# lightonai/next-plaid

Measured on AMD Instinct MI355X. Metric: queries/sec + p50 latency, k=10, 10M-doc x 300-tok x d128 PLAID index, 1/2/4/8 GPU, higher is better.
Workload: dtype f32 (split-bf16 hi/lo MFMA on the residual term of MaxSim, f32-class accuracy)

## Files before the change

### next-plaid_amd/csrc/np_kernels.h

```cpp
#pragma once
#include <hip/hip_runtime.h>
#include <stdint.h>

namespace np {

typedef float f32x16 __attribute__((ext_vector_type(16)));
typedef __bf16 bf16x8 __attribute__((ext_vector_type(8)));

#define NP_NEG_INF (-__builtin_huge_valf())
#define NP_MAX_QT 8

__device__ __forceinline__ uint32_t okey(float x) {
  uint32_t b = __float_as_uint(x);
  uint32_t k = (b & 0x80000000u) ? ~b : (b | 0x80000000u);
  return ((b & 0x7F800000u) == 0x7F800000u) ? 0u : k;
}
__device__ __forceinline__ float unkey(uint32_t k) {
  uint32_t b = (k & 0x80000000u) ? (k ^ 0x80000000u) : ~k;
  return __uint_as_float(b);
}
__device__ __forceinline__ bool finitef(float x) { return (__float_as_uint(x) & 0x7F800000u) != 0x7F800000u; }
__device__ __forceinline__ float readlane_f(float v, int lane) {
  return __int_as_float(__builtin_amdgcn_readlane(__float_as_int(v), lane));
}
// ... 2011 lines not shown
    const uint4* metab = cand_meta + pbase;
    for (int64_t tile0 = 0; tile0 < n; tile0 += NG * NP_S4S_MAXD) {
      const int d = (int)min((int64_t)NP_S4S_MAXD, (n - tile0 + NG - 1) / NG);
      __syncthreads();
      for (int k = 0; k < d; ++k) {
        const int64_t i = tile0 + (int64_t)k * NG + gid;
        s_state[k][tid] = make_float4(NP_NEG_INF, NP_NEG_INF, NP_NEG_INF, NP_NEG_INF);
        if (jq == 0) {
          int64_t off = 0;
          uint4 sg = make_uint4(0, 0, 0, 0);
          if (i < n) {
            const uint4 m = metab[i];
            off = (int64_t)m.z | ((int64_t)(m.w & 0xFF) << 32);
            sg = useg[m.x];
            toks += (unsigned long long)(m.w >> 8);
            ucnt += (unsigned long long)m.y;
          }
          s_off[k][g] = off;
          *reinterpret_cast<uint4*>(&s_end[k][g][0]) = sg;
        }
      }
      __syncthreads();
      for (int p = 0; p < P; ++p) {
        int len = 0;
        int64_t abs0 = 0;
        if (jq < d) {
          const int e = (int)s_end[jq][g][((p + 1) << pshift) - 1];
          const int s = p ? (int)s_end[jq][g][(p << pshift) - 1] : 0;
          len = e - s;
          abs0 = s_off[jq][g] + s;
        }
        const int pad = (len + 3) & ~3;
        int incl = pad;
#pragma unroll
        for (int o = 1; o < LPR; o <<= 1) {
          const int v = __shfl_up(incl, o, LPR);
          if (jq >= o) incl += v;
        }
        if (jq < NP_S4S_MAXD) {
          s_pfx[g][jq] = incl - pad;
          s_abs[g][jq] = abs0;
          s_len[g][jq] = len;
        }
        const int Lg = __shfl(incl, lbase + LPR - 1);
        int maxL = Lg;
#pragma unroll
        for (int o = LPR; o < 64; o <<= 1) maxL = max(maxL, __shfl_xor(maxL, o));
        maxL = __builtin_amdgcn_readfirstlane(maxL);
        __builtin_amdgcn_fence(__ATOMIC_RELEASE, "wavefront");
        __builtin_amdgcn_wave_barrier();
        const int p1 = s_pfx[g][1], p2 = s_pfx[g][2], p3 = s_pfx[g][3], p4 = s_pfx[g][4];
        const uint32_t slice_lo = (uint32_t)(p << pshift) * slice_w;
        const char* Tp = Tb + (size_t)slice_lo * row_bytes;
        for (int base = 0; base < maxL; base += NP_S4S_CAP) {
#pragma unroll
          for (int h = 0; h < 2; ++h) {
            uint32_t cv[NST / 2];
#pragma unroll
            for (int i = 0; i < NST / 2; ++i) {
              const int pos = base + jq + LPR * (h * (NST / 2) + i);
              const int slot = (pos >= p1) + (pos >= p2) + (pos >= p3) + (pos >= p4);
              const int idx = min(pos - s_pfx[g][slot], max(s_len[g][slot] - 1, 0));
              int64_t a = s_abs[g][slot] + (int64_t)max(idx, 0);
              a = (pos < Lg) ? min(a, T - 1) : 0;
              cv[i] = codes[a];
            }
#pragma unroll
            for (int i = 0; i < NST / 2; ++i) {
              const int w = jq + LPR * (h * (NST / 2) + i);
              const int pos = base + w;
              const bool valid = pos < Lg;
              const int slot = (pos >= p1) + (pos >= p2) + (pos >= p3) + (pos >= p4);
              s_codes[g][w] = valid ? (uint16_t)(cv[i] - slice_lo) : (uint16_t)0;
              if ((pos & 3) == 0) s_slot[g][w >> 2] = valid ? (uint8_t)slot : (uint8_t)NP_S4S_MAXD;
            }
          }
          __builtin_amdgcn_fence(__ATOMIC_RELEASE, "wavefront");
          __builtin_amdgcn_wave_barrier();
          const int nwin = min(NP_S4S_CAP, maxL - base);
          for (int t0 = 0; t0 < nwin; t0 += 8) {
            const bool two = t0 + 4 < nwin;
            const uint2 ca = *reinterpret_cast<const uint2*>(&s_codes[g][t0]);
            const int sa = (int)s_slot[g][t0 >> 2];
            float4 v[8];
            v[0] = *reinterpret_cast<const float4*>(Tp + ((ca.x & 0xFFFFu) * row_bytes + col_bytes));
            v[1] = *reinterpret_cast<const float4*>(Tp + ((ca.x >> 16) * row_bytes + col_bytes));
            v[2] = *reinterpret_cast<const float4*>(Tp + ((ca.y & 0xFFFFu) * row_bytes + col_bytes));
            v[3] = *reinterpret_cast<const float4*>(Tp + ((ca.y >> 16) * row_bytes + col_bytes));
            int sb = NP_S4S_MAXD;
            if (two) {
              const uint2 cb = *reinterpret_cast<const uint2*>(&s_codes[g][t0 + 4]);
              sb = (int)s_slot[g][(t0 + 4) >> 2];
              v[4] = *reinterpret_cast<const float4*>(Tp + ((cb.x & 0xFFFFu) * row_bytes + col_bytes));
              v[5] = *reinterpret_cast<const float4*>(Tp + ((cb.x >> 16) * row_bytes + col_bytes));
              v[6] = *reinterpret_cast<const float4*>(Tp + ((cb.y & 0xFFFFu) * row_bytes + col_bytes));
              v[7] = *reinterpret_cast<const float4*>(Tp + ((cb.y >> 16) * row_bytes + col_bytes));
            } else {
#pragma unroll
              for (int u = 4; u < 8; ++u) v[u] = make_float4(NP_NEG_INF, NP_NEG_INF, NP_NEG_INF, NP_NEG_INF);
            }
            s4_fence<8>(v);
            float4 ma = s_state[sa][tid];
#pragma unroll
            for (int u = 0; u < 4; ++u) {
              ma.x = fmaxf(ma.x, v[u].x);
              ma.y = fmaxf(ma.y, v[u].y);
              ma.z = fmaxf(ma.z, v[u].z);
              ma.w = fmaxf(ma.w, v[u].w);
            }
            s_state[sa][tid] = ma;
            float4 mb = s_state[sb][tid];
#pragma unroll
            for (int u = 4; u < 8; ++u) {
              mb.x = fmaxf(mb.x, v[u].x);
              mb.y = fmaxf(mb.y, v[u].y);
              mb.z = fmaxf(mb.z, v[u].z);
              mb.w = fmaxf(mb.w, v[u].w);
            }
            s_state[sb][tid] = mb;
          }
          __builtin_amdgcn_fence(__ATOMIC_RELEASE, "wavefront");
          __builtin_amdgcn_wave_barrier();
        }
      }
      for (int k = 0; k < d; ++k) {
        const int64_t i = tile0 + (int64_t)k * NG + gid;
        const float4 m = s_state[k][tid];
        float score = 0.f;
        for (int jj = 0; 4 * jj < lq; ++jj) {
          const float a0 = __shfl(m.x, lbase + jj), a1 = __shfl(m.y, lbase + jj);
          const float a2 = __shfl(m.z, lbase + jj), a3 = __shfl(m.w, lbase + jj);
          if (a0 > NP_NEG_INF) score += a0;
          if (4 * jj + 1 < lq && a1 > NP_NEG_INF) score += a1;
          if (4 * jj + 2 < lq && a2 > NP_NEG_INF) score += a2;
          if (4 * jj + 3 < lq && a3 > NP_NEG_INF) score += a3;
        }
        if (jq == 0 && i < n) approx[pbase + i] = s_end[k][g][7] ? score : 0.f;
      }
    }
  }
#pragma unroll
  for (int o = 32; o > 0; o >>= 1) {
    toks += __shfl_xor(toks, o);
    ucnt += __shfl_xor(ucnt, o);
  }
  if (lane == 0 && toks && ctr) {
    atomicAdd(&ctr->n_cand_tokens, toks);
    atomicAdd(&ctr->n_cand_codes, ucnt);
  }
}

#define NP_UB_NBX 96

template <int ROWB, typename CT, int MODE, int FLOOR = 0>
__global__ void __launch_bounds__(256) approx_ub_kernel(const uint8_t* __restrict__ QCU, int64_t KP,
                                                        const uint4* __restrict__ cand_meta ,
                                                        const int32_t* __restrict__ n_begin ,
                                                        const int32_t* __restrict__ n_count ,
                                                        const int32_t* __restrict__ n_cand ,
                                                        RoundPlan rp, int round,
                                                        int max_rounds, const CT* __restrict__ codes ,
                                                        const uint32_t* __restrict__ qflag, int n_sel,
                                                        uint16_t* __restrict__ U ,
                                                        uint32_t* __restrict__ hist , int hshift,
                                                        uint32_t* __restrict__ cursor ,
                                                        int32_t* __restrict__ slots ,
                                                        int32_t* __restrict__ ticket , int B,
                                                        int steal_min ,
                                                        Counters* ctr, int count_tokens ,
                                                        int direct_wpq ,
                                                        int static_claims ,
                                                        const uint32_t* __restrict__ warmbits = nullptr ,
                                                        const uint32_t* __restrict__ lam2_b = nullptr ,
                                                        const int32_t* __restrict__ qoff = nullptr ) {
  static_assert(FLOOR == 0 || (MODE == 2 && ROWB <= 64), "the floored level: bounds-checked loads");
  constexpr bool WLDS = FLOOR && sizeof(CT) == 2;
  constexpr int LPD = ROWB / 16;
  constexpr int DPW = 64 / LPD;
  constexpr int CAP = sizeof(CT) == 2 ? 128 : 64;
  constexpr int CPS = CAP / 32;
  constexpr bool NT = MODE == 1, OOB = MODE == 2;
  static_assert(ROWB == 32 || ROWB == 64 || ROWB == 128 || ROWB == 256, "row = power-of-two bytes >= LQP");
  __shared__ uint32_t s_hist[NP_UB_BINS];
  __shared__ CT s_codes[4][DPW][CAP];
  __shared__ uint32_t s_warm[WLDS ? 2048 : 4];
  __shared__ int s_ndk[4][FLOOR ? DPW : 1];
  __shared__ int64_t s_cl[4][DPW];
  __shared__ int s_nd[4][DPW];
  const int tid = threadIdx.x, lane = tid & 63, wave = tid >> 6;
  const int jl = lane & (LPD - 1), grp = lane / LPD;
  const int x = blockIdx.x & 7;
  if (round >= rp.round_tab[2 * max_rounds]) return;
  const int rb = rp.round_tab[2 * round], re = rp.round_tab[2 * round + 1];
  unsigned long long toks = 0, ucnt = 0, ndoc = 0;
  const int half = lane >> 5, hl = lane & 31;
  __shared__ int s_q;
  for (int step = 0;; ++step) {
    __syncthreads();
    if (direct_wpq > 0) {
      if (step > 0) break;
      const int j = rb + (int)blockIdx.x / direct_wpq;
      if (j >= re) break;
      if (tid == 0) s_q = rp.order[j];
    } else if (tid == 0)
      s_q = xcd_next_query(slots, ticket, x, step, B, rp.order, rb, re, [&]() {
        int best = -3;
        if (static_claims) return best;
        int64_t most = steal_min;
        for (int j = rb; j < re; ++j) {
          const int b2 = rp.order[j];
          if (qflag[b2] || n_cand[b2] <= n_sel) continue;
          const int64_t n2 = n_count[b2];
          const int64_t left = n2 - (int64_t)__hip_atomic_load(&cursor[b2], __ATOMIC_RELAXED, __HIP_MEMORY_SCOPE_AGENT);
          if (left >= most) {
            most = left;
            best = b2;
          }
        }
        return best;
      });
    __syncthreads();
    const int b = __builtin_amdgcn_readfirstlane(s_q);
    if (b < 0) break;
    if (qflag[b] || n_cand[b] <= n_sel) continue;
    const int64_t first = n_begin ? n_begin[b] : 0;
    const int64_t n = n_count[b];
    if (n <= 0) continue;
    const int64_t pbase = rp.cand_base[b] + first;
    const uint4* metab = cand_meta + pbase;
    const char* Tb = reinterpret_cast<const char*>(QCU + (int64_t)b * KP * ROWB) + jl * 16;
    const uint64_t tb64 = reinterpret_cast<uint64_t>(QCU + (int64_t)b * KP * ROWB);
    const uint32_t tlo = (uint32_t)__builtin_amdgcn_readfirstlane((int)(uint32_t)tb64);
    const uint32_t thi = (uint32_t)__builtin_amdgcn_readfirstlane((int)(uint32_t)(tb64 >> 32));
    const __amdgpu_buffer_rsrc_t trs = __builtin_amdgcn_make_buffer_rsrc(
        reinterpret_cast<void*>(((uint64_t)thi << 32) | tlo), 0, (int)(KP * ROWB), 0x00020000);
    uint32_t* hb = hist ? hist + (int64_t)b * NP_UB_BINS : nullptr;
    __syncthreads();
    if (hb)
      for (int i = tid; i < NP_UB_BINS; i += 256) s_hist[i] = 0;
    uint32_t lam2 = 0;
    int Lq = 0;
    const uint32_t* wb = nullptr;
    if constexpr (FLOOR) {
      wb = warmbits + (int64_t)b * (KP >> 5);
      if constexpr (WLDS)
        for (int i = tid; i < 2048; i += 256) s_warm[i] = i < (int)(KP >> 5) ? wb[i] : 0u;
      lam2 = lam2_b[b];
      Lq = qoff[b + 1] - qoff[b];
    }
    __syncthreads();
    const int64_t NWS = direct_wpq > 0 ? (int64_t)direct_wpq * 4 : (int64_t)(gridDim.x >> 3) * 4;
    const int64_t gw = direct_wpq > 0 ? (int64_t)((int)blockIdx.x % direct_wpq) * 4 + wave : (int64_t)(blockIdx.x >> 3) * 4 + wave;
    int64_t istat = gw * DPW;
    uint32_t inext = 0;
    if (!static_claims && lane == 0) inext = atomicAdd(&cursor[b], (uint32_t)DPW);
    for (;;) {
      const int64_t i0 = static_claims ? istat : (int64_t)(uint32_t)__builtin_amdgcn_readfirstlane((int)inext);
      if (i0 >= n) break;
      istat += NWS * DPW;
      if (!static_claims && lane == 0) inext = atomicAdd(&cursor[b], (uint32_t)DPW);
      const int64_t i = i0 + grp;
      const bool valid = i < n;
      uint4 m;
      if constexpr (NT) {
        const uint32_t* mp = reinterpret_cast<const uint32_t*>(metab + (valid ? i : n - 1));
        m = make_uint4(__builtin_nontemporal_load(mp), __builtin_nontemporal_load(mp + 1), __builtin_nontemporal_load(mp + 2),
                       __builtin_nontemporal_load(mp + 3));
      } else {
        m = metab[valid ? i : n - 1];
      }
      const int nd = valid ? (int)m.y : 0;
      const int64_t cl = (int64_t)m.z | ((int64_t)(m.w & 0xFF) << 32);
      if (jl == 0) {
        s_cl[wave][grp] = cl;
        s_nd[wave][grp] = nd;
        if (valid) {
          toks += (unsigned long long)(m.w >> 8);
          if constexpr (!FLOOR) ucnt += (unsigned long long)nd;
          ++ndoc;
        }
      }
      int nmax = nd;
#pragma unroll
      for (int o = LPD; o < 64; o <<= 1) nmax = max(nmax, __shfl_xor(nmax, o));
      nmax = __builtin_amdgcn_readfirstlane(nmax);
      uint32_t st[16];
#pragma unroll
      for (int k = 0; k < 16; ++k) st[k] = 0;
      for (int p0 = 0; p0 < nmax; p0 += CAP) {
        __builtin_amdgcn_fence(__ATOMIC_RELEASE, "wavefront");
        __builtin_amdgcn_wave_barrier();
        constexpr int SB = DPW / 2 < 8 ? DPW / 2 : 8;
#pragma unroll 1
        for (int sb = 0; sb < DPW / 2; sb += SB) {
          uint32_t cv[SB][4], c0[SB], wvg[(FLOOR && !WLDS) ? SB : 1][CPS];
          int nds[SB];
#pragma unroll
          for (int j = 0; j < SB; ++j) {
            const int sl = 2 * (sb + j) + half;
            nds[j] = s_nd[wave][sl];
            const CT* cp = codes + s_cl[wave][sl];
            const int pos = min(p0 + CPS * hl, max(nds[j] - 1, 0) & ~(CPS - 1));
            if constexpr (NT) {
              c0[j] = (uint32_t)__builtin_nontemporal_load(cp);
#pragma unroll
              for (int k = 0; k < CPS; ++k) cv[j][k] = (uint32_t)__builtin_nontemporal_load(cp + pos + k);
            } else {
              c0[j] = (uint32_t)cp[0];
              const uint2 raw = *reinterpret_cast<const uint2*>(cp + pos);
              if constexpr (sizeof(CT) == 2) {
                cv[j][0] = raw.x & 0xFFFFu; cv[j][1] = raw.x >> 16; cv[j][2] = raw.y & 0xFFFFu; cv[j][3] = raw.y >> 16;
              } else {
                cv[j][0] = raw.x; cv[j][1] = raw.y;
              }
            }
          }
          if constexpr (FLOOR && !WLDS) {
            const uint32_t wlast = (uint32_t)(KP >> 5) - 1u;
#pragma unroll
            for (int j = 0; j < SB; ++j)
#pragma unroll
              for (int k = 0; k < CPS; ++k)
                wvg[j][k] = (p0 + CPS * hl + k < nds[j]) ? wb[min(cv[j][k] >> 5, wlast)] : 0u;
          }
#pragma unroll
          for (int j = 0; j < SB; ++j) {
            const int sl = 2 * (sb + j) + half;
            const int pos = p0 + CPS * hl;
            if constexpr (FLOOR) {
              uint32_t wv[CPS];
#pragma unroll
              for (int k = 0; k < CPS; ++k) {
                if constexpr (WLDS) wv[k] = s_warm[(cv[j][k] >> 5) & 0x7FFu];
                else wv[k] = wvg[j][k];
              }
              int base = 0;
              CT* dstc = &s_codes[wave][sl][0];
#pragma unroll
              for (int k = 0; k < CPS; ++k) {
                const bool kp = pos + k < nds[j] && ((wv[k] >> (cv[j][k] & 31u)) & 1u) != 0u;
                const unsigned long long bal = __ballot(kp);
                const uint32_t hm = half ? (uint32_t)(bal >> 32) : (uint32_t)bal;
                if (kp) dstc[base + (int)__popc(hm & ((1u << hl) - 1u))] = (CT)cv[j][k];
                base += (int)__popc(hm);
              }
              if (hl == 0) s_ndk[wave][sl] = base;
              __builtin_amdgcn_sched_barrier(0);
              continue;
            }
#pragma unroll
            for (int k = 0; k < CPS; ++k)
              if (pos + k >= nds[j]) cv[j][k] = c0[j];
            CT* dst = &s_codes[wave][sl][CPS * hl];
            if constexpr (sizeof(CT) == 2) {
              *reinterpret_cast<uint2*>(dst) = make_uint2(cv[j][0] | (cv[j][1] << 16), cv[j][2] | (cv[j][3] << 16));
            } else {
              *reinterpret_cast<uint2*>(dst) = make_uint2(cv[j][0], cv[j][1]);
            }
          }
        }
        __builtin_amdgcn_fence(__ATOMIC_RELEASE, "wavefront");
        __builtin_amdgcn_wave_barrier();
        int np = (min(CAP, nmax - p0) + 7) & ~7;
        int ndk = 0;
        if constexpr (FLOOR) {
          ndk = s_ndk[wave][grp];
          if (jl == 0 && valid) ucnt += (unsigned long long)ndk;
          int km = ndk;
#pragma unroll
          for (int o = LPD; o < 64; o <<= 1) km = max(km, __shfl_xor(km, o));
          np = (__builtin_amdgcn_readfirstlane(km) + 7) & ~7;
        }
        const CT* mine = &s_codes[wave][grp][0];
        auto issue = [&](int t, uint4 (&v)[8]) {
          uint32_t c[8];
          if constexpr (sizeof(CT) == 2) {
            const uint4 cw = *reinterpret_cast<const uint4*>(mine + t);
            c[0] = cw.x & 0xFFFFu; c[1] = cw.x >> 16; c[2] = cw.y & 0xFFFFu; c[3] = cw.y >> 16;
            c[4] = cw.z & 0xFFFFu; c[5] = cw.z >> 16; c[6] = cw.w & 0xFFFFu; c[7] = cw.w >> 16;
          } else {
            const uint4 ca = *reinterpret_cast<const uint4*>(mine + t), cb = *reinterpret_cast<const uint4*>(mine + t + 4);
            c[0] = ca.x; c[1] = ca.y; c[2] = ca.z; c[3] = ca.w;
            c[4] = cb.x; c[5] = cb.y; c[6] = cb.z; c[7] = cb.w;
          }
          if constexpr (OOB) {
            typedef uint32_t u32x4 __attribute__((ext_vector_type(4)));
#pragma unroll
            for (int k = 0; k < 8; ++k) {
              const bool live = FLOOR ? (t + k < ndk) : (p0 + t + k < nd);
              const uint32_t off = live ? c[k] * (uint32_t)ROWB + (uint32_t)(jl * 16) : 0x7FFFFFF0u;
              const u32x4 r = __builtin_amdgcn_raw_buffer_load_b128(trs, (int)off, 0, 0);
              v[k] = make_uint4(r.x, r.y, r.z, r.w);
            }
          } else {
#pragma unroll
            for (int k = 0; k < 8; ++k) v[k] = *reinterpret_cast<const uint4*>(Tb + (size_t)c[k] * ROWB);
          }
        };
        auto fold = [&](uint4 (&v)[8]) {
          asm volatile("" : "+v"(v[0].x), "+v"(v[1].x), "+v"(v[2].x), "+v"(v[3].x), "+v"(v[4].x), "+v"(v[5].x), "+v"(v[6].x), "+v"(v[7].x));
#pragma unroll
          for (int k = 0; k < 8; ++k) {
            const uint32_t w4[4] = {v[k].x, v[k].y, v[k].z, v[k].w};
#pragma unroll
            for (int j = 0; j < 4; ++j)
#pragma unroll
              for (int e = 0; e < 4; ++e) st[4 * j + e] = max(st[4 * j + e], (w4[j] >> (8 * e)) & 0xFFu);
          }
        };
        uint4 va[8], vb[8];
        issue(0, va);
        int t = 0;
        for (; t + 16 < np; t += 16) {
          issue(t + 8, vb);
          fold(va);
          issue(t + 16, va);
          fold(vb);
        }
        if (t + 8 < np) {
          issue(t + 8, vb);
          fold(va);
          fold(vb);
        } else {
          fold(va);
        }
      }
      uint32_t sum = 0;
      int slo = 0;
      if constexpr (FLOOR) {
        uint32_t fl = lam2;
        int lq_here = Lq - 16 * jl;
        asm volatile("" : "+v"(fl), "+v"(lq_here));
#pragma unroll
        for (int k = 0; k < 16; ++k) {
          slo += (int)st[k] - ((k < lq_here && st[k] <= 1u) ? 254 : 0);
          sum += max(st[k], k < lq_here ? fl : 0u);
        }
      } else {
#pragma unroll
        for (int k = 0; k < 16; ++k) {
          sum += st[k];
          slo += (int)st[k] - (st[k] == 1u ? 254 : 0);
        }
      }
#pragma unroll
      for (int o = 1; o < LPD; o <<= 1) {
        sum += (uint32_t)__shfl_xor((int)sum, o);
        slo += __shfl_xor(slo, o);
      }
      const uint32_t sum_lo = (uint32_t)max(slo, 0);
      if (valid && jl == 0) {
        U[pbase + i] = (uint16_t)sum;
        if (hb) atomicAdd(&s_hist[min(sum_lo >> hshift, (uint32_t)(NP_UB_BINS - 1))], 1u);
      }
      __builtin_amdgcn_wave_barrier();
    }
    __syncthreads();
    if (hb)
      for (int i = tid; i < NP_UB_BINS; i += 256) {
        const uint32_t v = s_hist[i];
        if (v) atomicAdd(&hb[i], v);
      }
  }
#pragma unroll
  for (int o = 32; o > 0; o >>= 1) {
    toks += __shfl_xor(toks, o);
    ucnt += __shfl_xor(ucnt, o);
    ndoc += __shfl_xor(ndoc, o);
  }
  __shared__ unsigned long long s_cnt[3];
  __syncthreads();
  if (tid == 0) s_cnt[0] = s_cnt[1] = s_cnt[2] = 0;
  __syncthreads();
  if (lane == 0 && toks) {
    atomicAdd(&s_cnt[0], toks);
    atomicAdd(&s_cnt[1], ucnt);
    atomicAdd(&s_cnt[2], ndoc);
  }
  __syncthreads();
  if (tid == 0 && s_cnt[0] && ctr) {
    if (count_tokens) {
      atomicAdd(&ctr->n_cand_tokens, s_cnt[0]);
      atomicAdd(&ctr->n_cand_dcodes, s_cnt[1]);
    } else {
      atomicAdd(&ctr->n_level2, s_cnt[2]);
    }
    atomicAdd(&ctr->n_cand_codes, s_cnt[1]);
  }
}

__global__ void __launch_bounds__(256) ub_thr_kernel(const uint32_t* __restrict__ hist, int hshift, int slack, int n_sel,
                                                     const int32_t* __restrict__ n_cand, RoundPlan rp, int round,
                                                     const uint32_t* __restrict__ qflag, uint32_t* __restrict__ thr) {
  __shared__ uint32_t s_part[256];
  constexpr int BPT = NP_UB_BINS / 256;
  const int b = blockIdx.x, tid = threadIdx.x;
  if (rp.round_of[b] != round) return;
  if (qflag[b] != 0 || n_cand[b] <= n_sel) {
    if (tid == 0) thr[b] = 0;
    return;
  }
  const uint32_t* hb = hist + (int64_t)b * NP_UB_BINS;
  const int top = (255 - tid) * BPT;
  uint32_t mine = 0;
#pragma unroll
  for (int k4 = 0; k4 < BPT / 4; ++k4) {
    const uint4 v = *reinterpret_cast<const uint4*>(hb + top + 4 * k4);
    mine += v.x + v.y + v.z + v.w;
  }
  s_part[tid] = mine;
  __syncthreads();
  if (tid == 0) {
    uint32_t cum = 0;
    int t = 0;
    for (; t < 255; ++t) {
      if (cum + s_part[t] >= (uint32_t)n_sel) break;
      cum += s_part[t];
    }
    int bin = (255 - t) * BPT + BPT - 1;
    for (; bin > (255 - t) * BPT; --bin) {
      if (cum + hb[bin] >= (uint32_t)n_sel) break;
      cum += hb[bin];
    }
    thr[b] = (uint32_t)max(0, bin - ((slack + (1 << hshift) - 1) >> hshift));
  }
}

struct CutP {
  const uint4* src;
  const int32_t* n_src_a;
  const int32_t* n_src_b;
  const uint16_t* U;
  const uint32_t* lo;
  const uint32_t* hi;
  int zero_mode;
  const uint4* all_src;
  const int32_t* n_all;
  uint4* dst;
  const int32_t* dst_begin;
  int32_t* n_dst;
  int hshift;
  Counters* ctr;
};

__global__ void __launch_bounds__(256) ub_cut_kernel(CutP p, RoundPlan rp, int round) {
  __shared__ int s_wcnt[4], s_base;
  __shared__ unsigned long long s_cnt[2];
  const int b = blockIdx.y, tid = threadIdx.x, lane = tid & 63, wave = tid >> 6;
  if (rp.round_of[b] != round) return;
  const uint32_t lo = p.lo[b], hi = p.hi ? p.hi[b] : 0xFFFFFFFFu;
  const bool all = lo == 0;
  if (all && p.zero_mode == 1) return;
  const uint4* src = all ? p.all_src : p.src;
  const int64_t n = all ? (int64_t)p.n_all[b] : (int64_t)p.n_src_a[b] + (p.n_src_b ? p.n_src_b[b] : 0);
  const int64_t pbase = rp.cand_base[b];
  const int64_t dbase = pbase + (p.dst_begin ? p.dst_begin[b] : 0);
  if (tid == 0) s_cnt[0] = s_cnt[1] = 0;
  unsigned long long toks = 0, ucnt = 0;
  constexpr int PT = 8;
  for (int64_t i0 = (int64_t)blockIdx.x * (256 * PT); i0 < n; i0 += (int64_t)gridDim.x * (256 * PT)) {
    bool keep[PT];
    unsigned long long bal[PT];
    int wtot = 0;
#pragma unroll
    for (int k = 0; k < PT; ++k) {
      const int64_t i = i0 + k * 256 + tid;
      bool kp = i < n;
      if (kp && !all) {
        const uint32_t bin = min((uint32_t)p.U[pbase + i] >> p.hshift, (uint32_t)(NP_UB_BINS - 1));
        kp = bin >= lo && bin < hi;
      }
      keep[k] = kp;
      bal[k] = __ballot(kp);
      wtot += (int)__popcll(bal[k]);
    }
    if (lane == 0) s_wcnt[wave] = wtot;
    __syncthreads();
    if (tid == 0) {
      const int tot = s_wcnt[0] + s_wcnt[1] + s_wcnt[2] + s_wcnt[3];
      s_base = tot ? atomicAdd(&p.n_dst[b], tot) : 0;
    }
    __syncthreads();
    int pos = s_base;
    for (int k = 0; k < wave; ++k) pos += s_wcnt[k];
#pragma unroll
    for (int k = 0; k < PT; ++k) {
      if (keep[k]) {
        const uint4 m = src[pbase + i0 + k * 256 + tid];
        p.dst[dbase + pos + (int)__popcll(bal[k] & ((1ull << lane) - 1ull))] = m;
        if (all) {
          toks += (unsigned long long)(m.w >> 8);
          ucnt += (unsigned long long)m.y;
        }
      }
      pos += (int)__popcll(bal[k]);
    }
    __syncthreads();
  }
  if (all && p.ctr) {
#pragma unroll
    for (int o = 32; o > 0; o >>= 1) {
      toks += __shfl_xor(toks, o);
      ucnt += __shfl_xor(ucnt, o);
    }
    if (lane == 0 && toks) {
      atomicAdd(&s_cnt[0], toks);
      atomicAdd(&s_cnt[1], ucnt);
    }
    __syncthreads();
    if (tid == 0 && s_cnt[0]) {
      atomicAdd(&p.ctr->n_cand_tokens, s_cnt[0]);
      atomicAdd(&p.ctr->n_cand_dcodes, s_cnt[1]);
      atomicAdd(&p.ctr->n_cand_codes, s_cnt[1]);
    }
  }
}

__global__ void __launch_bounds__(256) hot_prep_kernel(const uint8_t* __restrict__ QCU, int64_t K, int64_t KP, int RB,
                                                       uint8_t* __restrict__ cmaxu ,
                                                       uint32_t* __restrict__ chist ) {
  __shared__ uint32_t s_h[256];
  const int b = blockIdx.y, tid = threadIdx.x;
// ... 2466 lines not shown
```

### next-plaid_amd/csrc/np_search.hip

```cpp
#include "np_internal.h"
#include "np_kernels.h"

#include <algorithm>
#include <array>
#include <cmath>
#include <stdlib.h>
#include <string.h>
#include <type_traits>
#include <utility>

namespace np {

struct Workspace {
  DevBuf q, qoff, Qt, Qb, Qbl, QCT, gmax, tauq, cellbits, cells_tmp, cells, n_cells, docbits, chunk_counts, cand, cand_meta, approx, n_cand,
      cand_base, round_of, round_tab, QCU, qinv, qflag, ub, ub_hist, ub_thr, ub_cursor, q_order, xcd_slots, surv_meta, n_surv, n_list2, sel_keys, sel_doc, nsel, exact, out_ids, out_scores, out_keys, out_counts, ctr, subset,
      subset_bits, elig, misc, cut, cmaxu, chist, ub2, ub_hist2, ub_thr2, list_meta, n_l1, n_l2, qpad, planes, levels, hotbits,
      gain, gsmall, ghist, s0_meta, s0_u, gacc, gdeep;
  void* h_pin = nullptr;
  size_t h_pin_cap = 0;
  unsigned long long* h_gain = nullptr;
  uint64_t h_gain_key = 0;
  hipEvent_t done = nullptr;
  bool done_valid = false;
  static constexpr int NBUF = 66;
// ... 1807 lines not shown
int np::encode_tokens_impl(const np_index* ix, const float* embeddings, int64_t n_tokens, int32_t dim,
                           const float* bucket_cutoffs, int64_t* out_codes, uint8_t* out_packed, float* out_norms) {
  if (!ix || n_tokens < 0 || (n_tokens > 0 && (!embeddings || !out_codes || !out_packed)) || !bucket_cutoffs) {
    set_error("encode_tokens: invalid argument");
    return NP_ERR_INVALID_ARGUMENT;
  }
  if (dim != ix->ldim) {
    set_error("Shape error: embedding dim %d does not match index dim %d", dim, ix->ldim);
    return NP_ERR_SHAPE;
  }
  if (!dim_supported(ix->dim, ix->nbits)) {
    set_error("Shape error: the HIP path supports dim <= 128; index has dim=%d nbits=%d", ix->ldim, ix->lnbits);
    return NP_ERR_SHAPE;
  }
  if (ix->K <= 0) {
    set_error("Codec error: the index has no centroids");
    return NP_ERR_CODEC;
  }
  if (n_tokens == 0) return NP_OK;
  DeviceGuard g(ix->device);
  CallState cs;
  NP_TRY(acquire_context(ix, &cs.ctx));
  UseGuard guard{ix, &cs};
  Workspace& w = *cs.ctx->ws;
  NP_TRY(begin_use(&cs, nullptr));
  guard.began = true;
  hipStream_t st = cs.stream;
  const int LQP = 32;
  const int64_t KP = ix->KP, G = KP >> 5;
  int64_t S = ix->ws_budget.load(std::memory_order_relaxed) / std::max<int64_t>(per_query_bytes(ix, LQP, 1, 1), 1);
  S = std::max<int64_t>(1, std::min<int64_t>(S, std::min<int64_t>(ix->opts.max_batch, NP_S4_MAXB)));
  S = std::min<int64_t>(S, (n_tokens + LQP - 1) / LQP);
  const int64_t TB = S * LQP;
  const int pd = ix->lpd, ncut = (1 << ix->lnbits) - 1;
  const int sdim = ix->dim;
  NP_TRY(w.q.reserve((size_t)TB * dim * 4));
  if (sdim != dim) NP_TRY(w.qpad.reserve((size_t)TB * sdim * 4));
  NP_TRY(w.qoff.reserve((size_t)(S + 1) * 4));
  NP_TRY(w.Qt.reserve((size_t)S * sdim * LQP * 4));
  NP_TRY(w.Qb.reserve((size_t)S * sdim * LQP * 2));
  NP_TRY(w.Qbl.reserve((size_t)S * sdim * LQP * 2));
  NP_TRY(w.QCT.reserve((size_t)S * KP * LQP * 4));
  NP_TRY(w.gmax.reserve((size_t)S * G * LQP * 4));
  NP_TRY(w.out_ids.reserve((size_t)TB * 8));
  NP_TRY(w.cand.reserve((size_t)TB * pd));
  NP_TRY(w.misc.reserve(std::max<size_t>(64, (size_t)ncut * 4)));
  if (out_norms) NP_TRY(w.approx.reserve((size_t)TB * 4));
  NP_HIP(hipMemcpyAsync(w.misc.p, bucket_cutoffs, (size_t)ncut * 4, hipMemcpyHostToDevice, st));
  std::vector<int32_t> h_off((size_t)S + 1);
  for (int64_t t0 = 0; t0 < n_tokens; t0 += TB) {
    const int64_t nb = std::min<int64_t>(TB, n_tokens - t0);
    const int Sb = (int)((nb + LQP - 1) / LQP);
    for (int s = 0; s <= Sb; ++s) h_off[(size_t)s] = (int32_t)std::min<int64_t>((int64_t)s * LQP, nb);
    NP_HIP(hipMemcpyAsync(w.q.p, embeddings + t0 * dim, (size_t)nb * dim * 4, hipMemcpyHostToDevice, st));
    NP_HIP(hipMemcpyAsync(w.qoff.p, h_off.data(), (size_t)(Sb + 1) * 4, hipMemcpyHostToDevice, st));
    const float* xs = w.q.as<float>();
    if (sdim != dim) {
      pad_rows_kernel<<<(unsigned)((nb * sdim + 255) / 256), 256, 0, st>>>(w.q.as<float>(), nb, dim, sdim, w.qpad.as<float>());
      xs = w.qpad.as<float>();
    }
    prep_queries_kernel<<<Sb, 256, 0, st>>>(xs, w.qoff.as<int32_t>(), sdim, LQP, w.Qt.as<float>(),
                                            w.Qb.as<__bf16>(), w.Qbl.as<__bf16>(), 0.f, nullptr, nullptr);
    launch_gemm(st, ix, w.Qt.as<float>(), Sb, LQP, w.QCT.as<float>(), w.gmax.as<uint32_t>());
    encode_argmax_kernel<<<(unsigned)((nb + 3) / 4), 256, 0, st>>>(w.QCT.as<float>(), w.gmax.as<uint32_t>(), ix->K, KP,
                                                                  LQP, nb, w.out_ids.as<int64_t>());
    encode_pack_kernel<<<(unsigned)((nb * pd + 255) / 256), 256, 0, st>>>(w.q.as<float>(), ix->d_centroids.get(),
                                                                         w.out_ids.as<int64_t>(), w.misc.as<float>(), nb,
                                                                         dim, sdim, ix->lnbits, w.cand.as<uint8_t>());
    if (out_norms)
      encode_norm_kernel<<<(unsigned)((nb + 255) / 256), 256, 0, st>>>(w.q.as<float>(), ix->d_centroids.get(), w.out_ids.as<int64_t>(),
                                                                        nb, dim, sdim, w.approx.as<float>());
    NP_HIP(hipGetLastError());
    NP_HIP(hipMemcpyAsync(out_codes + t0, w.out_ids.p, (size_t)nb * 8, hipMemcpyDeviceToHost, st));
    NP_HIP(hipMemcpyAsync(out_packed + t0 * pd, w.cand.p, (size_t)nb * pd, hipMemcpyDeviceToHost, st));
    if (out_norms) NP_HIP(hipMemcpyAsync(out_norms + t0, w.approx.p, (size_t)nb * 4, hipMemcpyDeviceToHost, st));
    NP_HIP(hipStreamSynchronize(st));
  }
  NP_TRY(end_use(&cs));
  return NP_OK;
}

extern "C" {

int np_hip_rerank_maxsim(int32_t device, const float* query, int32_t n_query_tokens, int32_t dim,
                         const float* doc_embeddings, const int64_t* doc_tok_offsets, int64_t n_docs, float* out_scores,
                         int64_t* out_order) {
  clear_error();
  if (n_docs <= 0) {
    set_error("No documents provided");
    return NP_ERR_INVALID_ARGUMENT;
  }
  if (!query || !doc_tok_offsets || !out_scores || n_query_tokens < 0 || dim <= 0) {
    set_error("rerank_maxsim: invalid argument");
    return NP_ERR_INVALID_ARGUMENT;
  }
  if (dim > 1024) {
    set_error("Shape error: rerank supports dim <= 1024, got %d", dim);
    return NP_ERR_SHAPE;
  }
  for (int64_t i = 0; i < n_docs; ++i)
    if (doc_tok_offsets[i + 1] < doc_tok_offsets[i] || doc_tok_offsets[0] != 0) {
      set_error("rerank_maxsim: doc_tok_offsets must start at 0 and be non-decreasing");
      return NP_ERR_INVALID_ARGUMENT;
    }
  const int64_t T = doc_tok_offsets[n_docs];
  if (T > 0 && !doc_embeddings) {
    set_error("rerank_maxsim: invalid argument");
    return NP_ERR_INVALID_ARGUMENT;
  }
  int ndev = 0;
  if (hipGetDeviceCount(&ndev) != hipSuccess || device < 0 || device >= ndev) {
    (void)hipGetLastError();
    set_error("no usable gfx950 device %d", device);
    return NP_ERR_DEVICE_UNAVAILABLE;
  }
  DeviceGuard g(device);
  DevPtr<float> d_q, d_d, d_s;
  DevPtr<int64_t> d_off;
  DevPtr<int> d_f;
  NP_TRY(d_q.alloc((size_t)n_query_tokens * dim));
  NP_TRY(d_d.alloc((size_t)T * dim));
  NP_TRY(d_s.alloc((size_t)n_docs));
  NP_TRY(d_off.alloc((size_t)n_docs + 1));
  NP_TRY(d_f.alloc((size_t)n_docs));
  if (n_query_tokens > 0) NP_HIP(hipMemcpy(d_q.get(), query, (size_t)n_query_tokens * dim * 4, hipMemcpyHostToDevice));
  if (T > 0) NP_HIP(hipMemcpy(d_d.get(), doc_embeddings, (size_t)T * dim * 4, hipMemcpyHostToDevice));
  NP_HIP(hipMemcpy(d_off.get(), doc_tok_offsets, (size_t)(n_docs + 1) * 8, hipMemcpyHostToDevice));
  rerank_kernel<<<(unsigned)n_docs, 256, (size_t)8 * dim * 4>>>(d_q.get(), n_query_tokens, dim, d_d.get(), d_off.get(), d_s.get(),
                                                                d_f.get());
  NP_HIP(hipGetLastError());
  std::vector<int> flags((size_t)n_docs);
  NP_HIP(hipMemcpy(out_scores, d_s.get(), (size_t)n_docs * 4, hipMemcpyDeviceToHost));
  NP_HIP(hipMemcpy(flags.data(), d_f.get(), (size_t)n_docs * 4, hipMemcpyDeviceToHost));
  for (int64_t i = 0; i < n_docs; ++i)
    if (flags[(size_t)i]) {
      set_error("Rerank score contains non-finite value");
      return NP_ERR_INVALID_ARGUMENT;
    }
  if (out_order) {
    auto key = [](float x) {
      uint32_t b;
      memcpy(&b, &x, 4);
      return (b & 0x80000000u) ? ~b : (b | 0x80000000u);
    };
    std::vector<int64_t> ord((size_t)n_docs);
    for (int64_t i = 0; i < n_docs; ++i) ord[(size_t)i] = i;
    std::stable_sort(ord.begin(), ord.end(),
                     [&](int64_t a, int64_t b) { return key(out_scores[a]) > key(out_scores[b]); });
    memcpy(out_order, ord.data(), (size_t)n_docs * 8);
  }
  return NP_OK;
}

}
```

Measured before the change: 20440.

## Pipeline query draw and candidate metadata prefetch in approx_ub_kernel

```diff
diff --git a/next-plaid_amd/csrc/np_kernels.h b/next-plaid_amd/csrc/np_kernels.h
--- a/next-plaid_amd/csrc/np_kernels.h
+++ b/next-plaid_amd/csrc/np_kernels.h
@@ -2187,6 +2187,15 @@
 
 #define NP_UB_NBX 96
 
+#ifdef NP_DIAGNOSTICS
+__device__ unsigned long long np_ub_stamps[32];
+#define NP_UB_CLK() ((long long)wall_clock64())
+#define NP_UB_ACC(k, v) (ub_acc[k] += (unsigned long long)(v))
+#else
+#define NP_UB_CLK() 0ll
+#define NP_UB_ACC(k, v) ((void)0)
+#endif
+
 template <int ROWB, typename CT, int MODE, int FLOOR = 0>
 __global__ void __launch_bounds__(256) approx_ub_kernel(const uint8_t* __restrict__ QCU, int64_t KP,
                                                         const uint4* __restrict__ cand_meta ,
@@ -2215,6 +2224,7 @@
   constexpr int CAP = sizeof(CT) == 2 ? 128 : 64;
   constexpr int CPS = CAP / 32;
   constexpr bool NT = MODE == 1, OOB = MODE == 2;
+  constexpr bool PRE = OOB && sizeof(CT) == 2;
   static_assert(ROWB == 32 || ROWB == 64 || ROWB == 128 || ROWB == 256, "row = power-of-two bytes >= LQP");
   __shared__ uint32_t s_hist[NP_UB_BINS];
   __shared__ CT s_codes[4][DPW][CAP];
@@ -2229,39 +2239,95 @@
   const int rb = rp.round_tab[2 * round], re = rp.round_tab[2 * round + 1];
   unsigned long long toks = 0, ucnt = 0, ndoc = 0;
   const int half = lane >> 5, hl = lane & 31;
-  __shared__ int s_q;
+  const uint32_t NWS = direct_wpq > 0 ? (uint32_t)direct_wpq * 4u : (gridDim.x >> 3) * 4u;
+  const uint32_t gw = direct_wpq > 0 ? (blockIdx.x % (uint32_t)direct_wpq) * 4u + wave : (blockIdx.x >> 3) * 4u + wave;
+  const uint32_t stat_end = static_claims ? 0u : NWS * DPW;
+  __shared__ int s_nx[2][8];
+  __shared__ int s_drew[2];
+  auto post = [&](int v, int* nx) {
+    const int bq = v <= -4 ? -4 - v : v;
+    int nn = 0;
+    if (bq >= 0) {
+      const uint32_t fl = qflag[bq];
+      const int nc = n_cand[bq], cnt = n_count[bq], beg = n_begin ? n_begin[bq] : 0;
+      const int64_t pb = rp.cand_base[bq] + beg;
+      if constexpr (FLOOR) {
+        nx[4] = (int)lam2_b[bq];
+        nx[5] = qoff[bq + 1] - qoff[bq];
+      }
+      nx[2] = (int)(uint32_t)pb;
+      nx[3] = (int)(pb >> 32);
+      if (!fl && nc > n_sel) nn = max(cnt, 0);
+    }
+    nx[1] = nn;
+    nx[0] = v;
+  };
+  auto draw = [&](int step_n) {
+    const int v = xcd_next_query(slots, ticket, x, step_n, B, rp.order, rb, re, [&]() {
+      int best = -3;
+      if (static_claims) return best;
+      int64_t most = steal_min;
+      for (int j = rb; j < re; ++j) {
+        const int b2 = rp.order[j];
+        if (qflag[b2] || n_cand[b2] <= n_sel) continue;
+        const int64_t n2 = n_count[b2];
+        const int64_t left =
+            n2 - (int64_t)stat_end - (int64_t)__hip_atomic_load(&cursor[b2], __ATOMIC_RELAXED, __HIP_MEMORY_SCOPE_AGENT);
+        if (left >= most) {
+          most = left;
+          best = -4 - b2;
+        }
+      }
+      return best;
+    });
+    post(v, s_nx[step_n & 1]);
+  };
+  if (tid == 0) {
+    s_drew[0] = s_drew[1] = 0;
+    if (direct_wpq > 0) {
+      const int j = rb + (int)blockIdx.x / direct_wpq;
+      post(j < re ? rp.order[j] : -3, s_nx[0]);
+      s_nx[1][0] = -3;
+    } else {
+      draw(0);
+    }
+  }
+  if (hist)
+    for (int i = tid; i < NP_UB_BINS; i += 256) s_hist[i] = 0;
+  uint32_t* hprev = nullptr;
+#ifdef NP_DIAGNOSTICS
+  unsigned long long ub_acc[10] = {0, 0, 0, 0, 0, 0, 0, 0, 0, 0};
+  long long t_idle = 0;
+#endif
   for (int step = 0;; ++step) {
     __syncthreads();
-    if (direct_wpq > 0) {
-      if (step > 0) break;
-      const int j = rb + (int)blockIdx.x / direct_wpq;
-      if (j >= re) break;
-      if (tid == 0) s_q = rp.order[j];
-    } else if (tid == 0)
-      s_q = xcd_next_query(slots, ticket, x, step, B, rp.order, rb, re, [&]() {
-        int best = -3;
-        if (static_claims) return best;
-        int64_t most = steal_min;
-        for (int j = rb; j < re; ++j) {
-          const int b2 = rp.order[j];
-          if (qflag[b2] || n_cand[b2] <= n_sel) continue;
-          const int64_t n2 = n_count[b2];
-          const int64_t left = n2 - (int64_t)__hip_atomic_load(&cursor[b2], __ATOMIC_RELAXED, __HIP_MEMORY_SCOPE_AGENT);
-          if (left >= most) {
-            most = left;
-            best = b2;
-          }
-        }
-        return best;
-      });
-    __syncthreads();
-    const int b = __builtin_amdgcn_readfirstlane(s_q);
-    if (b < 0) break;
-    if (qflag[b] || n_cand[b] <= n_sel) continue;
-    const int64_t first = n_begin ? n_begin[b] : 0;
-    const int64_t n = n_count[b];
-    if (n <= 0) continue;
-    const int64_t pbase = rp.cand_base[b] + first;
+    [[maybe_unused]] const long long t_a = NP_UB_CLK();
+#ifdef NP_DIAGNOSTICS
+    if (t_idle) NP_UB_ACC(4, t_a - t_idle);
+    t_idle = 0;
+#endif
+    const int* nx = s_nx[step & 1];
+    const int slotv = __builtin_amdgcn_readfirstlane(nx[0]);
+    const uint32_t n = (uint32_t)__builtin_amdgcn_readfirstlane(nx[1]);
+    if (hprev)
+      for (int i = tid; i < NP_UB_BINS; i += 256) {
+        const uint32_t v = s_hist[i];
+        if (v) {
+          atomicAdd(&hprev[i], v);
+          s_hist[i] = 0;
+        }
+      }
+    hprev = nullptr;
+    if (slotv < 0 && slotv > -4) break;
+    if (tid == 0) s_drew[(step + 1) & 1] = 0;
+    if (n == 0) {
+      if (tid == 0 && direct_wpq <= 0) draw(step + 1);
+      continue;
+    }
+    const bool joined = slotv <= -4;
+    const int b = joined ? -4 - slotv : slotv;
+    const int64_t pbase = ((int64_t)__builtin_amdgcn_readfirstlane(nx[3]) << 32) |
+                          (int64_t)(uint32_t)__builtin_amdgcn_readfirstlane(nx[2]);
     const uint4* metab = cand_meta + pbase;
     const char* Tb = reinterpret_cast<const char*>(QCU + (int64_t)b * KP * ROWB) + jl * 16;
     const uint64_t tb64 = reinterpret_cast<uint64_t>(QCU + (int64_t)b * KP * ROWB);
@@ -2270,9 +2336,24 @@
     const __amdgpu_buffer_rsrc_t trs = __builtin_amdgcn_make_buffer_rsrc(
         reinterpret_cast<void*>(((uint64_t)thi << 32) | tlo), 0, (int)(KP * ROWB), 0x00020000);
     uint32_t* hb = hist ? hist + (int64_t)b * NP_UB_BINS : nullptr;
-    __syncthreads();
-    if (hb)
-      for (int i = tid; i < NP_UB_BINS; i += 256) s_hist[i] = 0;
+    auto load_rec = [&](uint32_t c0) {
+      const uint32_t ir = min(c0 + (uint32_t)grp, n - 1u);
+      if constexpr (NT) {
+        const uint32_t* mp = reinterpret_cast<const uint32_t*>(metab + ir);
+        return make_uint4(__builtin_nontemporal_load(mp), __builtin_nontemporal_load(mp + 1), __builtin_nontemporal_load(mp + 2),
+                          __builtin_nontemporal_load(mp + 3));
+      } else {
+        return metab[ir];
+      }
+    };
+    uint32_t i0 = gw * DPW;
+    uint32_t inext = 0;
+    if (!static_claims && joined) {
+      if (lane == 0) inext = atomicAdd(&cursor[b], (uint32_t)DPW);
+      i0 = stat_end + (uint32_t)__builtin_amdgcn_readfirstlane((int)inext);
+    }
+    uint4 m = make_uint4(0u, 0u, 0u, 0u);
+    if (i0 < n) m = load_rec(i0);
     uint32_t lam2 = 0;
     int Lq = 0;
     const uint32_t* wb = nullptr;
@@ -2280,30 +2361,25 @@
       wb = warmbits + (int64_t)b * (KP >> 5);
       if constexpr (WLDS)
         for (int i = tid; i < 2048; i += 256) s_warm[i] = i < (int)(KP >> 5) ? wb[i] : 0u;
-      lam2 = lam2_b[b];
-      Lq = qoff[b + 1] - qoff[b];
+      lam2 = (uint32_t)__builtin_amdgcn_readfirstlane(nx[4]);
+      Lq = __builtin_amdgcn_readfirstlane(nx[5]);
     }
     __syncthreads();
-    const int64_t NWS = direct_wpq > 0 ? (int64_t)direct_wpq * 4 : (int64_t)(gridDim.x >> 3) * 4;
-    const int64_t gw = direct_wpq > 0 ? (int64_t)((int)blockIdx.x % direct_wpq) * 4 + wave : (int64_t)(blockIdx.x >> 3) * 4 + wave;
-    int64_t istat = gw * DPW;
-    uint32_t inext = 0;
-    if (!static_claims && lane == 0) inext = atomicAdd(&cursor[b], (uint32_t)DPW);
-    for (;;) {
-      const int64_t i0 = static_claims ? istat : (int64_t)(uint32_t)__builtin_amdgcn_readfirstlane((int)inext);
-      if (i0 >= n) break;
-      istat += NWS * DPW;
+    NP_UB_ACC(0, NP_UB_CLK() - t_a);
+    NP_UB_ACC(6, 1);
+    if (i0 >= n) NP_UB_ACC(7, 1);
+    while (i0 < n) {
+      [[maybe_unused]] const long long t_c0 = NP_UB_CLK();
+      [[maybe_unused]] long long t_c1 = t_c0, t_c2 = t_c0;
       if (!static_claims && lane == 0) inext = atomicAdd(&cursor[b], (uint32_t)DPW);
-      const int64_t i = i0 + grp;
+      uint32_t i0n = n;
+      uint4 mn = make_uint4(0u, 0u, 0u, 0u);
+      auto prefetch = [&]() {
+        i0n = static_claims ? i0 + NWS * DPW : stat_end + (uint32_t)__builtin_amdgcn_readfirstlane((int)inext);
+        if (i0n < n) mn = load_rec(i0n);
+      };
+      const uint32_t i = i0 + (uint32_t)grp;
       const bool valid = i < n;
-      uint4 m;
-      if constexpr (NT) {
-        const uint32_t* mp = reinterpret_cast<const uint32_t*>(metab + (valid ? i : n - 1));
-        m = make_uint4(__builtin_nontemporal_load(mp), __builtin_nontemporal_load(mp + 1), __builtin_nontemporal_load(mp + 2),
-                       __builtin_nontemporal_load(mp + 3));
-      } else {
-        m = metab[valid ? i : n - 1];
-      }
       const int nd = valid ? (int)m.y : 0;
       const int64_t cl = (int64_t)m.z | ((int64_t)(m.w & 0xFF) << 32);
       if (jl == 0) {
@@ -2325,58 +2401,67 @@
       for (int p0 = 0; p0 < nmax; p0 += CAP) {
         __builtin_amdgcn_fence(__ATOMIC_RELEASE, "wavefront");
         __builtin_amdgcn_wave_barrier();
-        constexpr int SB = DPW / 2 < 8 ? DPW / 2 : 8;
+        constexpr int SB = (OOB && sizeof(CT) == 2) ? DPW / 2 : (DPW / 2 < 8 ? DPW / 2 : 8);
 #pragma unroll 1
         for (int sb = 0; sb < DPW / 2; sb += SB) {
-          uint32_t cv[SB][4], c0[SB], wvg[(FLOOR && !WLDS) ? SB : 1][CPS];
-          int nds[SB];
+          uint2 rw[SB];
+          uint32_t c0[FLOOR ? 1 : SB], wvg[(FLOOR && !WLDS) ? SB : 1][CPS];
 #pragma unroll
           for (int j = 0; j < SB; ++j) {
             const int sl = 2 * (sb + j) + half;
-            nds[j] = s_nd[wave][sl];
+            const int ndj = s_nd[wave][sl];
             const CT* cp = codes + s_cl[wave][sl];
-            const int pos = min(p0 + CPS * hl, max(nds[j] - 1, 0) & ~(CPS - 1));
+            const int pos = min(p0 + CPS * hl, max(ndj - 1, 0) & ~(CPS - 1));
             if constexpr (NT) {
-              c0[j] = (uint32_t)__builtin_nontemporal_load(cp);
-#pragma unroll
-              for (int k = 0; k < CPS; ++k) cv[j][k] = (uint32_t)__builtin_nontemporal_load(cp + pos + k);
+              if constexpr (!FLOOR) c0[j] = (uint32_t)__builtin_nontemporal_load(cp);
+              const uint32_t* cw = reinterpret_cast<const uint32_t*>(cp + pos);
+              rw[j] = make_uint2(__builtin_nontemporal_load(cw), __builtin_nontemporal_load(cw + 1));
             } else {
-              c0[j] = (uint32_t)cp[0];
-              const uint2 raw = *reinterpret_cast<const uint2*>(cp + pos);
-              if constexpr (sizeof(CT) == 2) {
-                cv[j][0] = raw.x & 0xFFFFu; cv[j][1] = raw.x >> 16; cv[j][2] = raw.y & 0xFFFFu; cv[j][3] = raw.y >> 16;
-              } else {
-                cv[j][0] = raw.x; cv[j][1] = raw.y;
-              }
+              if constexpr (!FLOOR) c0[j] = (uint32_t)cp[0];
+              rw[j] = *reinterpret_cast<const uint2*>(cp + pos);
             }
           }
+          auto unpack = [&](int j, uint32_t (&cv)[4]) {
+            if constexpr (sizeof(CT) == 2) {
+              cv[0] = rw[j].x & 0xFFFFu; cv[1] = rw[j].x >> 16; cv[2] = rw[j].y & 0xFFFFu; cv[3] = rw[j].y >> 16;
+            } else {
+              cv[0] = rw[j].x; cv[1] = rw[j].y; cv[2] = cv[3] = 0;
+            }
+          };
           if constexpr (FLOOR && !WLDS) {
             const uint32_t wlast = (uint32_t)(KP >> 5) - 1u;
 #pragma unroll
-            for (int j = 0; j < SB; ++j)
+            for (int j = 0; j < SB; ++j) {
+              uint32_t cv[4];
+              unpack(j, cv);
+              const int ndj = s_nd[wave][2 * (sb + j) + half];
 #pragma unroll
               for (int k = 0; k < CPS; ++k)
-                wvg[j][k] = (p0 + CPS * hl + k < nds[j]) ? wb[min(cv[j][k] >> 5, wlast)] : 0u;
+                wvg[j][k] = (p0 + CPS * hl + k < ndj) ? wb[min(cv[k] >> 5, wlast)] : 0u;
+            }
           }
 #pragma unroll
           for (int j = 0; j < SB; ++j) {
             const int sl = 2 * (sb + j) + half;
             const int pos = p0 + CPS * hl;
+            const int ndj = s_nd[wave][sl];
+            uint32_t cv[4];
+            unpack(j, cv);
             if constexpr (FLOOR) {
               uint32_t wv[CPS];
 #pragma unroll
               for (int k = 0; k < CPS; ++k) {
-                if constexpr (WLDS) wv[k] = s_warm[(cv[j][k] >> 5) & 0x7FFu];
+                if constexpr (WLDS) wv[k] = s_warm[(cv[k] >> 5) & 0x7FFu];
                 else wv[k] = wvg[j][k];
               }
               int base = 0;
               CT* dstc = &s_codes[wave][sl][0];
 #pragma unroll
               for (int k = 0; k < CPS; ++k) {
-                const bool kp = pos + k < nds[j] && ((wv[k] >> (cv[j][k] & 31u)) & 1u) != 0u;
+                const bool kp = pos + k < ndj && ((wv[k] >> (cv[k] & 31u)) & 1u) != 0u;
                 const unsigned long long bal = __ballot(kp);
                 const uint32_t hm = half ? (uint32_t)(bal >> 32) : (uint32_t)bal;
-                if (kp) dstc[base + (int)__popc(hm & ((1u << hl) - 1u))] = (CT)cv[j][k];
+                if (kp) dstc[base + (int)__popc(hm & ((1u << hl) - 1u))] = (CT)cv[k];
                 base += (int)__popc(hm);
               }
               if (hl == 0) s_ndk[wave][sl] = base;
@@ -2385,17 +2470,20 @@
             }
 #pragma unroll
             for (int k = 0; k < CPS; ++k)
-              if (pos + k >= nds[j]) cv[j][k] = c0[j];
+              if (pos + k >= ndj) cv[k] = c0[j];
             CT* dst = &s_codes[wave][sl][CPS * hl];
             if constexpr (sizeof(CT) == 2) {
-              *reinterpret_cast<uint2*>(dst) = make_uint2(cv[j][0] | (cv[j][1] << 16), cv[j][2] | (cv[j][3] << 16));
+              *reinterpret_cast<uint2*>(dst) = make_uint2(cv[0] | (cv[1] << 16), cv[2] | (cv[3] << 16));
             } else {
-              *reinterpret_cast<uint2*>(dst) = make_uint2(cv[j][0], cv[j][1]);
+              *reinterpret_cast<uint2*>(dst) = make_uint2(cv[0], cv[1]);
             }
           }
         }
         __builtin_amdgcn_fence(__ATOMIC_RELEASE, "wavefront");
         __builtin_amdgcn_wave_barrier();
+        if constexpr (PRE)
+          if (p0 == 0) prefetch();
+        if (p0 == 0) t_c1 = NP_UB_CLK();
         int np = (min(CAP, nmax - p0) + 7) & ~7;
         int ndk = 0;
         if constexpr (FLOOR) {
@@ -2460,6 +2548,7 @@
           fold(va);
         }
       }
+      t_c2 = NP_UB_CLK();
       uint32_t sum = 0;
       int slo = 0;
       if constexpr (FLOOR) {
@@ -2489,13 +2578,30 @@
         if (hb) atomicAdd(&s_hist[min(sum_lo >> hshift, (uint32_t)(NP_UB_BINS - 1))], 1u);
       }
       __builtin_amdgcn_wave_barrier();
-    }
-    __syncthreads();
-    if (hb)
-      for (int i = tid; i < NP_UB_BINS; i += 256) {
-        const uint32_t v = s_hist[i];
-        if (v) atomicAdd(&hb[i], v);
-      }
+      if (!PRE || nmax == 0) prefetch();
+      i0 = i0n;
+      m = mn;
+#ifdef NP_DIAGNOSTICS
+      {
+        const long long t_c3 = NP_UB_CLK();
+        NP_UB_ACC(1, t_c1 - t_c0);
+        NP_UB_ACC(2, t_c2 - t_c1);
+        NP_UB_ACC(3, t_c3 - t_c2);
+        NP_UB_ACC(5, 1);
+      }
+#endif
+    }
+#ifdef NP_DIAGNOSTICS
+    t_idle = NP_UB_CLK();
+#endif
+    if (direct_wpq <= 0 && lane == 0 && atomicAdd(&s_drew[step & 1], 1) == 0) {
+      draw(step + 1);
+#ifdef NP_DIAGNOSTICS
+      NP_UB_ACC(8, NP_UB_CLK() - t_idle);
+      NP_UB_ACC(9, 1);
+#endif
+    }
+    hprev = hb;
   }
 #pragma unroll
   for (int o = 32; o > 0; o >>= 1) {
@@ -2503,6 +2609,11 @@
     ucnt += __shfl_xor(ucnt, o);
     ndoc += __shfl_xor(ndoc, o);
   }
+#ifdef NP_DIAGNOSTICS
+  if (lane == 0)
+    for (int k = 0; k < 10; ++k)
+      if (ub_acc[k]) atomicAdd(&np_ub_stamps[(direct_wpq > 0 ? 16 : 0) + k], ub_acc[k]);
+#endif
   __shared__ unsigned long long s_cnt[3];
   __syncthreads();
   if (tid == 0) s_cnt[0] = s_cnt[1] = s_cnt[2] = 0;
diff --git a/next-plaid_amd/csrc/np_search.hip b/next-plaid_amd/csrc/np_search.hip
--- a/next-plaid_amd/csrc/np_search.hip
+++ b/next-plaid_amd/csrc/np_search.hip
@@ -1983,4 +1983,14 @@
   return NP_OK;
 }
 
-}
+
+#ifdef NP_DIAGNOSTICS
+int np_hip_diag_ub_stamps(unsigned long long* out, int reset) {
+  if (hipDeviceSynchronize() != hipSuccess) return NP_ERR_SEARCH;
+  unsigned long long zero[32] = {};
+  if (out && hipMemcpyFromSymbol(out, HIP_SYMBOL(np::np_ub_stamps), sizeof(zero)) != hipSuccess) return NP_ERR_SEARCH;
+  if (reset && hipMemcpyToSymbol(HIP_SYMBOL(np::np_ub_stamps), zero, sizeof(zero)) != hipSuccess) return NP_ERR_SEARCH;
+  return NP_OK;
+}
+#endif
+}
```

Measured after the change: 20250. Within noise of the previous version (-0.9%).
